# StarsX/FluidX12

Measured on AMD Instinct MI355X. Metric: voxel-updates/sec (advect+40 Jacobi) at 256^3; achieved HBM GB/s vs peak, higher is better.
Workload: dtype f32

## Files before the change

### fluidx12_amd/csrc/fx_jacobi_strip4.hip

```cpp
#include "fx_internal.h"
#include "fx_pk.h"
#include <algorithm>
#include <climits>
#include <cstdlib>

namespace fx {

namespace {

#ifndef FX_STRIP4_OUTER_ROWS
#define FX_STRIP4_OUTER_ROWS 3
#endif
constexpr int NRO = FX_STRIP4_OUTER_ROWS;
constexpr int NRI = 8 - NRO;

template <int NR_, bool A_, bool W_, int NW_ = 4, int XS_ = 0, bool NT_ = false, bool XT_ = false> struct Role4 {
	static constexpr int NR = NR_;
	static constexpr bool XT = XT_;
	static constexpr bool NT = NT_;
	static constexpr int NW = NW_;
	static constexpr int XS = XS_;
	static constexpr int XO1 = 0, XO2 = (A_ || W_) ? 4 : 2, XO3 = (A_ || W_) ? 3 : 4;
	static constexpr bool A = A_, W = W_;
	static constexpr int NI = NR + (A ? 4 : 1) + (W ? 4 : 1);
// ... 35 lines not shown
	fx_f2 lx = XS == 2 ? pk_mov_sel<HI, 0>(E, c01) : pk_mov(c01, c01, 0);
	const fx_f2 mid = pk_mov(c01, c23, 1);
	fx_f2 rx = XS == 1 ? pk_mov_sel<1, HI>(c23, E) : pk_mov(c23, c23, 2);
	const float cx_ = c.x, cw_ = c.w, lx0_ = lx.x, rx1_ = rx.y;
	lx.x = __builtin_bit_cast(float, __builtin_amdgcn_update_dpp(__builtin_bit_cast(int, lx0_), __builtin_bit_cast(int, cw_), 0x138, 0xf, 0xf, false));
	rx.y = __builtin_bit_cast(float, __builtin_amdgcn_update_dpp(__builtin_bit_cast(int, rx1_), __builtin_bit_cast(int, cx_), 0x130, 0xf, 0xf, false));
	const fx_f2 b01 = { bb.x, bb.y }, b23 = { bb.z, bb.w }, U01 = { U.x, U.y }, U23 = { U.z, U.w }, D01 = { D.x, D.y }, D23 = { D.z, D.w };
	const fx_f2 F01 = { F.x, F.y }, F23 = { F.z, F.w }, B01 = { Bk.x, Bk.y }, B23 = { Bk.z, Bk.w };
	fx_f2 s01 = (((((lx - b01) + mid) + U01) + D01) + F01) + B01;
	fx_f2 s23 = (((((mid - b23) + rx) + U23) + D23) + F23) + B23;
	const float inv = __uint_as_float(0x3e2aaaabu);
	s01 *= inv; s23 *= inv;
	return v4f{ s01.x, s01.y, s23.x, s23.y };
}
template <int XS, int C>
__device__ __forceinline__ v4f relax4qe(v4f c, v4f U, v4f D, v4f F, v4f Bk, v4f bb, v4f EA, fx_f2 EB)
{
	static_assert(C >= 0 && C < 6, "six cut cells per step");
	const fx_f2 E = C < 2 ? fx_f2{ EA.x, EA.y } : C < 4 ? fx_f2{ EA.z, EA.w } : EB;
	return relax4qx<XS, C & 1>(c, U, D, F, Bk, bb, E);
}

__device__ __forceinline__ uint32_t opaque32q(uint32_t v) { asm volatile("" : "+v"(v)); return v; }
typedef __attribute__((address_space(1))) v4f g_v4f;
__device__ __forceinline__ void store_row4(char* base, uint32_t off, v4f v)
{
#ifdef FX_S4_SC1
	*(volatile g_v4f*)(g_v4f*)(base + off) = v;
#elif defined(FX_S4_NT)
	__builtin_nontemporal_store(v, reinterpret_cast<v4f*>(base + off));
#else
	*reinterpret_cast<v4f*>(base + off) = v;
#endif
}
__device__ __forceinline__ void store_row4nt(char* base, uint32_t off, v4f v)
{
	__builtin_nontemporal_store(v, reinterpret_cast<v4f*>(base + off));
}

typedef unsigned u4 __attribute__((ext_vector_type(4)));
template <bool NT>
__device__ __forceinline__ void store_row4xt(char* base, uint32_t off, bool keep, v4f v)
{
	const __amdgpu_buffer_rsrc_t rs = __builtin_amdgcn_make_buffer_rsrc(base, 0, 0x7fffffff, 0x00020000);
	const uint32_t o = keep ? off : 0xfffffff0u;
	__builtin_amdgcn_raw_buffer_store_b128(__builtin_bit_cast(u4, v), rs, (int)o, 0, NT ? 2 : 0);
// ... 80 lines not shown
	uint32_t act;
};

__device__ unsigned g_strip4_fault;
constexpr int kWaitSpins4 = 1 << 16;
__device__ __forceinline__ void strip4_raise_fault() { (void)__hip_atomic_fetch_or(&g_strip4_fault, 1u, __ATOMIC_RELAXED, __HIP_MEMORY_SCOPE_AGENT); }

__device__ __forceinline__ v4f lds_wait_read4(uint32_t flag_byte_addr, int need, uint32_t row_byte_addr)
{
	int f;
	v4f d;
	for (int spins = 0;; ++spins) {
		asm volatile("ds_read_b32 %0, %2\n\tds_read_b128 %1, %3\n\ts_waitcnt lgkmcnt(0)" : "=&v"(f), "=&v"(d) : "v"(flag_byte_addr), "v"(row_byte_addr) : "memory");
		if (f >= need) break;
		if (__builtin_expect(spins > kWaitSpins4, 0)) { strip4_raise_fault(); break; }
		__builtin_amdgcn_s_sleep(1);
	}
	return d;
}
__device__ __forceinline__ void lds_post4(uint32_t lds_byte_addr, int v)
{
	asm volatile("ds_write_b32 %0, %1" :: "v"(lds_byte_addr), "v"(v) : "memory");
}

template <class R> struct Strip4 {
	int s_ctr, s_old, s_b2, s_b3, s_b4;
	const char* pp; const char* pbq; char* po; char* po_zb;
	size_t plane_bytes;
	v4f* lds; v4f* xbuf; int* xflag;
	uint32_t xf0, xb0;
	int q, zb, ze, q_load_last, b_load_last, Zg, wave, lane;
	bool wall_top, wall_bot;
	bool keep;
	uint32_t eoff;
	float E0;
	v4f* xe;
	uint32_t xe0;
};
template <int NW> __device__ __forceinline__ constexpr int xeslot(int par, int w) { return (par * NW + w) * 2; }

template <int XS>
__device__ __forceinline__ void xe_publish(uint32_t slot_addr, uint32_t cnt_addr, int q, float v0, float v1, float v2, float v3, float v4, float v5)
{
	if (XS == 1)
		asm volatile("s_bfm_b64 exec, 1, 63\n\tds_write2_b32 %0, %2, %3 offset1:1\n\tds_write2_b32 %0, %4, %5 offset0:2 offset1:3\n\tds_write2_b32 %0, %6, %7 offset0:4 offset1:5\n\t"
			"ds_write_b32 %1, %8\n\ts_mov_b64 exec, -1" :: "v"(slot_addr), "v"(cnt_addr), "v"(v0), "v"(v1), "v"(v2), "v"(v3), "v"(v4), "v"(v5), "v"(q) : "memory");
	else
		asm volatile("s_mov_b64 exec, 1\n\tds_write2_b32 %0, %2, %3 offset1:1\n\tds_write2_b32 %0, %4, %5 offset0:2 offset1:3\n\tds_write2_b32 %0, %6, %7 offset0:4 offset1:5\n\t"
			"ds_write_b32 %1, %8\n\ts_mov_b64 exec, -1" :: "v"(slot_addr), "v"(cnt_addr), "v"(v0), "v"(v1), "v"(v2), "v"(v3), "v"(v4), "v"(v5), "v"(q) : "memory");
}
struct XMail { int f; v4f a; fx_f2 b; };
template <class R>
__device__ __forceinline__ void xe_fetch(const Strip4<R>& st, XMail& x)
// ... 2 lines not shown
	x.f = INT_MAX; return;
#endif
	const int wp = st.wave ^ 4, pr = (st.q - 1) & 1;
	x.f = __hip_atomic_load(reinterpret_cast<const int*>(st.xflag) + 3 * R::NW + wp, __ATOMIC_RELAXED, __HIP_MEMORY_SCOPE_WORKGROUP);
	asm volatile("" ::: "memory");
	__builtin_amdgcn_sched_barrier(0);
	x.a = st.xe[xeslot<R::NW>(pr, wp)];
	x.b = *reinterpret_cast<const fx_f2*>(st.xe + xeslot<R::NW>(pr, wp) + 1);
	asm volatile("" ::: "memory");
	__builtin_amdgcn_sched_barrier(0);
}
template <class R>
__device__ __forceinline__ void xe_check(const Strip4<R>& st, XMail& x)
{
	if (__builtin_expect(x.f < st.q - 1, 0)) {
		const int wp = st.wave ^ 4, pr = (st.q - 1) & 1;
		x.a = lds_wait_read4(st.xf0 + 4u * (uint32_t)(3 * R::NW + wp), st.q - 1, st.xe0 + 16u * (uint32_t)xeslot<R::NW>(pr, wp));
		x.b = *reinterpret_cast<const fx_f2*>(st.xe + xeslot<R::NW>(pr, wp) + 1);
	}
}
__device__ __forceinline__ float lane_cell(float v, int lane) { return __builtin_bit_cast(float, __builtin_amdgcn_readlane(__builtin_bit_cast(int, v), lane)); }

#define FXQ_LDS(st, slot, r) (st).lds[(slot) + (r) * 64]
#define FXQ_RARE_BRANCH asm volatile("; rare path")

template <class R> struct Mail4 { int fu, fd; v4f hu, hd; };

template <class R, int L>
__device__ __forceinline__ void mail_fetch4(const Strip4<R>& st, Mail4<R>& m)
{
#ifdef FX_S4_NOHAND
	return;
#endif
	const int q = st.q, w = st.wave, pr = (q - 1) & 1;
#ifdef FX_S4_BARRIER
	if (!R::A) m.hu = st.xbuf[xrow<R::NW>(pr, FX_WU(w), L - 1, 0) + st.lane];
	if (!R::W) m.hd = st.xbuf[xrow<R::NW>(pr, w, L - 1, 1) + st.lane];
	m.fu = m.fd = INT_MAX;
	return;
#endif
	const int* flags = reinterpret_cast<const int*>(st.xflag);
	if (!R::A) m.fu = __hip_atomic_load(flags + (L - 1) * R::NW + FX_WU(w), __ATOMIC_RELAXED, __HIP_MEMORY_SCOPE_WORKGROUP);
	if (!R::W) m.fd = __hip_atomic_load(flags + (L - 1) * R::NW + FX_WD(w), __ATOMIC_RELAXED, __HIP_MEMORY_SCOPE_WORKGROUP);
	asm volatile("" ::: "memory");
	__builtin_amdgcn_sched_barrier(0);
	if (!R::A) m.hu = st.xbuf[xrow<R::NW>(pr, FX_WU(w), L - 1, 0) + st.lane];
	if (!R::W) m.hd = st.xbuf[xrow<R::NW>(pr, w, L - 1, 1) + st.lane];
	asm volatile("" ::: "memory");
	__builtin_amdgcn_sched_barrier(0);
}

template <class R, int L, int NL>
__device__ __forceinline__ void hand_over4(const Strip4<R>& st, Mail4<R>& m, const v4f (&PN)[NL], v4f& HU, v4f& HD)
{
#ifdef FX_S4_NOHAND
	return;
#endif
	const int q = st.q, w = st.wave;
	const int pr = (q - 1) & 1, pw = q & 1;
	const v4f mine_top = PN[0], mine_bot = PN[NL - 1];
	if (!R::A) {
		if (__builtin_expect(m.fu < q - 1, 0)) m.hu = lds_wait_read4(st.xf0 + 4u * (uint32_t)((L - 1) * R::NW + FX_WU(w)), q - 1, st.xb0 + 16u * (uint32_t)(xrow<R::NW>(pr, FX_WU(w), L - 1, 0) + st.lane));
		HU = m.hu;
	}
	if (!R::W) {
		if (__builtin_expect(m.fd < q - 1, 0)) m.hd = lds_wait_read4(st.xf0 + 4u * (uint32_t)((L - 1) * R::NW + FX_WD(w)), q - 1, st.xb0 + 16u * (uint32_t)(xrow<R::NW>(pr, w, L - 1, 1) + st.lane));
		HD = m.hd;
	}
	asm volatile("" ::: "memory");
	if (!R::A) st.xbuf[xrow<R::NW>(pw, FX_WU(w), L - 1, 1) + st.lane] = mine_top;
	if (!R::W) st.xbuf[xrow<R::NW>(pw, w, L - 1, 0) + st.lane] = mine_bot;
#ifndef FX_S4_BARRIER
#ifdef FX_LAB_DROP_PUBLISH
	if (L == 2 && w == 3) return;
#endif
	if (st.lane == 0) lds_post4(st.xf0 + 4u * (uint32_t)((L - 1) * R::NW + w), q);
#endif
}

template <class R, int L, int NL, int NN, bool MK = false>
__device__ __forceinline__ void relax_level4(const Strip4<R>& st, const v4f (&Pold)[NL], const v4f (&Pctr)[NL], const v4f (&Pnew)[NL],
	const v4f (&Bq)[NN], v4f HU, v4f HD, v4f (&out)[NN], uint32_t mctr, uint32_t& mout, const XMail* xm = nullptr)
{
	constexpr int EOFF = L == 1 ? R::XO1 : L == 2 ? R::XO2 : R::XO3;
	static_assert(!(MK && R::XS), "the masked loop runs on whole-row waves");
	uint32_t m_ = 0u;
#pragma unroll
	for (int kk = 0; kk < NN; ++kk) {
		constexpr int UP = R::UP;
#ifdef FX_M_PLAIN
		const int k = kk;
#else
		const int k = MK ? NN - 1 - kk : kk;
#endif
		const int jc = k + UP;
		const v4f c = Pctr[jc];
		v4f u = jc >= 1 ? Pctr[jc >= 1 ? jc - 1 : 0] : HU;
		v4f d = jc + 1 < NL ? Pctr[jc + 1 < NL ? jc + 1 : 0] : HD;
		if (R::A && k == 3 - L && st.wall_top) u = c;
// ... 10 lines not shown
			switch (k) {
			case 0: out[k] = relax4qe<R::XS ? R::XS : 1, (EOFF + 0) % 6>(c, u, d, Pold[jc], Pnew[jc], Bq[k], xm->a, xm->b); break;
			case 1: out[k] = relax4qe<R::XS ? R::XS : 1, (EOFF + 1) % 6>(c, u, d, Pold[jc], Pnew[jc], Bq[k], xm->a, xm->b); break;
			default: out[k] = relax4qe<R::XS ? R::XS : 1, (EOFF + 2) % 6>(c, u, d, Pold[jc], Pnew[jc], Bq[k], xm->a, xm->b); break;
			}
		} else
			out[k] = relax4q(c, u, d, Pold[jc], Pnew[jc], Bq[k]);
	}
#ifdef FX_M_PLAIN
	if (MK) mout = m_;
#else
	if (MK) mout = ((mctr >> (4 * R::UP)) & ((1u << (4 * NN)) - 1u)) | m_;
#endif
}

template <class R>
__device__ __forceinline__ void frz_out4(const Strip4<R>& st, Frz4& fz, char* dst_, const v4f (&X_)[R::NR], uint32_t m4_, const uint32_t (&roff)[R::NI])
{
	constexpr int NR = R::NR, RB = R::A ? 4 : 1;
	const int z = st.q - 4;
	const ptrdiff_t mo_ = (dst_ - fz.outA) >> 4;
#ifndef FX_M_ONEP
#pragma unroll
	for (int m = 0; m < NR; ++m) store_row4(dst_ + fz.dB, opaque32q(roff[m + RB]), X_[m]);
#endif
#ifdef FX_M_NOBYTES
	if (st.q < -1000)
#endif
#pragma unroll
	for (int m = 0; m < NR; ++m) {
		const uint32_t o_ = opaque32q(roff[m + RB] >> 4);
		fz.mA[mo_ + o_] = (uint8_t)FXQ_NIB(m4_, m);
		fz.mB[mo_ + o_] = (uint8_t)FXQ_NIB(m4_, m);
	}
	if (z >= st.zb) {
#pragma unroll
		for (int m = 0; m < NR; ++m) if (FXQ_NIB(m4_, m) != 15u) { fz.rel |= 16u; fz.act |= 1u << m; }
		if ((z & 7) == 7 || z == st.ze - 1) {
#pragma unroll
			for (int m = 0; m < NR; ++m) {
				const unsigned long long bal_ = __ballot((fz.act >> m) & 1u);
				if ((st.lane & 7) == 0 && ((bal_ >> st.lane) & 0xFFull) != 0ull)
					fz.tile_mark[((z >> 3) * fz.nty + ((fz.y_own + m) >> 3)) * fz.ntx + (st.lane >> 3)] = fz.tag;
			}
			fz.act = 0u;
		}
	}
// ... 2 lines not shown
template <class R, int PH, bool S1, bool S2, bool S3, bool S4, bool MK = false>
__device__ __forceinline__ void step4(Strip4<R>& st, v4f (&P1)[3][R::N1], v4f (&P2)[3][R::N2], v4f (&P3)[3][R::N3], v4f (&NP)[R::NI], v4f (&NB)[R::N1], v4f (&NBn)[R::N1], v4f (&Bk)[R::N2], const uint32_t (&roff)[R::NI],
	Frz4& fz, uint32_t (&MW)[3][3], uint32_t (&NM)[R::N1])
{
	constexpr int NEW = PH % 3, CTR = (PH + 2) % 3, OLD = (PH + 1) % 3;
	constexpr int NI = R::NI, N1 = R::N1, N2 = R::N2, N3 = R::N3, NR = R::NR, UP = R::UP;
	static_assert(!MK || R::NW != 4, "the masked loop runs in the octet");
	constexpr int O1 = R::A ? 3 : 0, O2 = R::A ? 2 : 0, O3 = R::A ? 1 : 0;
	constexpr uint32_t OWN = (1u << (4 * NR)) - 1u;
	const int q = st.q;
	uint32_t M0n = 0u;
	if (MK) {
#pragma unroll
		for (int j = 0; j < N1; ++j) M0n |= (NM[j] & 15u) << (4 * j);
		if (q >= st.zb && q < st.ze && (~(M0n >> (4 * O1)) & OWN) != 0u) fz.rel |= 1u;
		if (q == 0) fz.M0c = M0n;
	}
	const v4f zero = v4f{ 0.0f, 0.0f, 0.0f, 0.0f };
	Mail4<R> M1, M2, M3;
	M1.fu = M1.fd = M2.fu = M2.fd = M3.fu = M3.fd = INT_MIN; M1.hu = M1.hd = M2.hu = M2.hd = M3.hu = M3.hd = zero;
#ifdef FX_S4_BARRIER
	asm volatile("s_waitcnt lgkmcnt(0)\n\ts_barrier" ::: "memory");
#endif
	if (S1) mail_fetch4<R, 1>(st, M1);
	XMail xm; xm.f = INT_MIN; xm.a = zero; xm.b = fx_f2{ 0.0f, 0.0f };
	if (R::XS && S2) xe_fetch<R>(st, xm);
#ifdef FX_S4_LATE_PREFETCH
	constexpr bool EARLY = false;
#else
	constexpr bool EARLY = R::NW == 4;
#endif
	constexpr bool LEAN = R::NW != 4;
	v4f NPc[EARLY ? NI : 1], NBc[EARLY ? N1 : 1];
	auto issue_prefetch = [&]() __attribute__((always_inline)) {
		if (!LEAN) {
#pragma unroll
			for (int j = 0; j < N1; ++j) NB[j] = NBn[j];
		}
#ifdef FX_S4_NOLOAD
		if (q + 1 <= st.b_load_last && q < -1000) {
#else
		if (LEAN ? q <= st.b_load_last : q + 1 <= st.b_load_last) {
#endif
#pragma unroll
			for (int j = 0; j < N1; ++j) (LEAN ? NB[j] : NBn[j]) = *reinterpret_cast<const v4f*>(st.pbq + opaque32q(roff[j + 1]));
		}
#ifdef FX_S4_NOLOAD
		if (q + 1 <= st.q_load_last && q < -1000) {
#else
		if (q + 1 <= st.q_load_last) {
#endif
#pragma unroll
			for (int i = 0; i < NI; ++i) NP[i] = *reinterpret_cast<const v4f*>(st.pp + opaque32q(roff[i]));
			if (MK) {
#pragma unroll
				for (int j = 0; j < N1; ++j) NM[j] = fz.pm[opaque32q(roff[j + 1] >> 4)];
			}
		}
		if (R::XS && q <= st.q_load_last) st.E0 = *reinterpret_cast<const float*>(st.pp - st.plane_bytes + st.eoff);
	};
	if (EARLY) {
#pragma unroll
		for (int i = 0; i < NI; ++i) NPc[i] = NP[i];
#pragma unroll
		for (int j = 0; j < N1; ++j) NBc[j] = NB[j];
		issue_prefetch();
	}
	auto np = [&](int i) __attribute__((always_inline)) -> v4f { return EARLY ? NPc[EARLY ? i : 0] : NP[i]; };
	auto nb = [&](int j) __attribute__((always_inline)) -> v4f { return EARLY ? NBc[EARLY ? j : 0] : NB[j]; };
	if (q == 0) {
#pragma unroll
		for (int i = 0; i < NI; ++i) FXQ_LDS(st, st.s_ctr, i) = np(i);
	}
	fx_f2 E1_[R::XS ? (N1 + 1) / 2 : 1];
	if (R::XS) {
#pragma unroll
		for (int j = 0; j < N1; ++j) { const float e_ = lane_cell(st.E0, j + 1); if (j & 1) E1_[j >> 1].y = e_; else E1_[j >> 1].x = e_; }
	}
	if (S1) {
		v4f T_[N1];
// ... 131 lines not shown
		}
#pragma unroll
		for (int m = 0; m < N3; ++m) P3[NEW][m] = T_[m];
		if (MK) MW[2][NEW] = m3_;
		if (__builtin_expect(q - 3 == 0, 0)) {
			FXQ_RARE_BRANCH;
#pragma unroll
			for (int m = 0; m < N3; ++m) P3[CTR][m] = T_[m];
			if (MK) MW[2][CTR] = m3_;
		}
	}
	v4f HU3 = zero, HD3 = zero;
	if (S3) hand_over4<R, 3, N3>(st, M3, P3[NEW], HU3, HD3);
	if (S4) {
		v4f X_[NR];
		uint32_t m4_ = 0u;
		relax_level4<R, 3, N3, NR, MK>(st, P3[OLD], P3[CTR], P3[NEW], B4_, HU3, HD3, X_, MK ? MW[2][CTR] : 0u, m4_, &xm);
		char* dst_ = q - 4 >= st.zb ? st.po : st.po_zb;
#ifdef FX_S4_NOSTORE
		if (q < -1000)
#endif
#pragma unroll
		for (int m = 0; m < NR; ++m) {
			if (R::XT) store_row4xt<R::NT>(dst_, opaque32q(roff[m + (R::A ? 4 : 1)]), st.keep, X_[m]);
			else if (R::NT) store_row4nt(dst_, opaque32q(roff[m + (R::A ? 4 : 1)]), X_[m]);
			else store_row4(dst_, opaque32q(roff[m + (R::A ? 4 : 1)]), X_[m]);
		}
		if (MK) frz_out4<R>(st, fz, dst_, X_, m4_, roff);
	}
#ifndef FX_S4_NOXE
	if (R::XS) {
		float v_[6] = { 0.0f, 0.0f, 0.0f, 0.0f, 0.0f, 0.0f };
#pragma unroll
		for (int k = 0; k < N2; ++k) v_[R::XO1 + k] = R::XS == 1 ? P1[NEW][k + UP].w : P1[NEW][k + UP].x;
#pragma unroll
		for (int k = 0; k < N3; ++k) v_[R::XO2 + k] = R::XS == 1 ? P2[NEW][k + UP].w : P2[NEW][k + UP].x;
#pragma unroll
		for (int k = 0; k < NR; ++k) v_[R::XO3 + k] = R::XS == 1 ? P3[NEW][k + UP].w : P3[NEW][k + UP].x;
		xe_publish<R::XS ? R::XS : 1>(st.xe0 + 16u * (uint32_t)xeslot<R::NW>(q & 1, st.wave), st.xf0 + 4u * (uint32_t)(3 * R::NW + st.wave), q, v_[0], v_[1], v_[2], v_[3], v_[4], v_[5]);
	}
#endif
	st.po += st.plane_bytes;
	++st.q;
}

template <class R, bool MK>
__device__ __forceinline__ void head_stores4(const Strip4<R>& st, const Frz4& fz, const uint32_t (&roff)[R::NI])
{
#ifndef FX_S4_NOHEADSTORES
	constexpr int RB = R::A ? 4 : 1;
	const v4f zero = v4f{ 0.0f, 0.0f, 0.0f, 0.0f };
#pragma unroll
	for (int m = 0; m < R::NR; ++m) {
		if (R::XT) store_row4xt<false>(st.po_zb, opaque32q(roff[m + RB]), st.keep, zero);
		else store_row4(st.po_zb, opaque32q(roff[m + RB]), zero);
	}
	if (MK) {
		const ptrdiff_t mo_ = (st.po_zb - fz.outA) >> 4;
#pragma unroll
		for (int m = 0; m < R::NR; ++m) store_row4(st.po_zb + fz.dB, opaque32q(roff[m + RB]), zero);
#pragma unroll
		for (int m = 0; m < R::NR; ++m) {
			const uint32_t o_ = opaque32q(roff[m + RB] >> 4);
			fz.mA[mo_ + o_] = (uint8_t)0;
			fz.mB[mo_ + o_] = (uint8_t)0;
		}
	}
#endif
}

template <class R, int NM_>
__device__ __forceinline__ void frz_begin4(const Geom& g, const FrzArgs& fa, const Strip4<R>& st, Frz4& fz, uint32_t (&MW)[3][3], uint32_t (&NM)[NM_],
	const uint32_t (&roff)[R::NI], float* p_out, int y0, int q0, bool fill)
{
	const size_t plane4 = st.plane_bytes >> 4;
	fz.outA = reinterpret_cast<char*>(p_out); fz.dB = reinterpret_cast<char*>(fa.p_outB) - reinterpret_cast<char*>(p_out);
	fz.mA = fa.m_outA; fz.mB = fa.m_outB; fz.tile_mark = fa.tile_mark; fz.tag = fa.tag; fz.ntx = fa.ntx; fz.nty = fa.nty; fz.y_own = y0;
	fz.M0c = 0u; fz.rel = 0u; fz.act = 0u;
#pragma unroll
	for (int l = 0; l < 3; ++l) MW[l][0] = MW[l][1] = MW[l][2] = 0u;
	const uint8_t* mb = fa.m_in + (size_t)g.lz(min(q0, st.q_load_last)) * plane4;
#pragma unroll
	for (int j = 0; j < NM_; ++j) NM[j] = mb[roff[j + 1] >> 4];
// ... 14 lines not shown
__device__ __forceinline__ void run4(const Geom& g, const float* __restrict__ p_in, const float* __restrict__ b, float* __restrict__ p_out,
	int zb, int ze, int y0, int wave, int lane, v4f* lds_slice, v4f* xbuf, int* xflag, const FrzArgs& fa, v4f* xe = nullptr, int x0 = 0, bool keep = true)
{
	Strip4<R> st;
	Frz4 fz;
	uint32_t MW[3][3], NM[R::N1];
#ifndef FX_O_NOPRIO
#ifndef FX_O_PRIO
#define FX_O_PRIO 2
#endif
	if (R::NW != 4) __builtin_amdgcn_s_setprio(FX_O_PRIO);
#endif
	v4f P1[3][R::N1], P2[3][R::N2], P3[3][R::N3], NP[R::NI], NB[R::N1], NBn[R::N1], Bk[R::N2];
	uint32_t roff[R::NI];
	const v4f zero = v4f{ 0.0f, 0.0f, 0.0f, 0.0f };
	const int qs = max(zb - 4, g.zlo), q_last = ze - 1 + 4;
	st.q_load_last = min(q_last, g.zhi);
	st.b_load_last = min(q_last - 1, g.zhi);
	st.zb = zb; st.ze = ze; st.Zg = g.Zg; st.wave = wave; st.lane = lane;
	st.wall_top = y0 == 0; st.wall_bot = y0 + R::NR >= g.Y;
	st.lds = lds_slice + lane; st.xbuf = xbuf; st.xflag = xflag;
	st.xf0 = (uint32_t)(size_t)(__attribute__((address_space(3))) int*)xflag;
	st.xb0 = (uint32_t)(size_t)(__attribute__((address_space(3))) v4f*)xbuf;
	const int yb = y0 - (R::A ? 4 : 1);
	const uint32_t XCOL = R::XT ? (uint32_t)x0 : R::XS == 2 ? 256u : 0u;
	st.keep = keep;
#pragma unroll
	for (int i = 0; i < R::NI; ++i) roff[i] = ((uint32_t)min(max(yb + i, 0), g.Y - 1) * (uint32_t)g.X + XCOL + 4u * (uint32_t)lane) * 4u;
	st.xe = xe; st.xe0 = (uint32_t)(size_t)(__attribute__((address_space(3))) v4f*)xe;
	st.eoff = ((uint32_t)min(max(yb + min(lane, R::NI - 1), 0), g.Y - 1) * (uint32_t)g.X + (R::XS == 2 ? 255u : 256u)) * 4u;
	st.E0 = 0.0f;
	st.s_ctr = 0; st.s_old = R::NI * 64;
	st.s_b2 = 2 * R::NI * 64; st.s_b3 = st.s_b2 + (R::NW == 4 ? R::N2 * 64 : 0); st.s_b4 = st.s_b3 + R::N2 * 64;
#pragma unroll
	for (int k = 0; k < 3; ++k) {
#pragma unroll
		for (int i = 0; i < R::N1; ++i) P1[k][i] = zero;
#pragma unroll
		for (int i = 0; i < R::N2; ++i) P2[k][i] = zero;
#pragma unroll
		for (int i = 0; i < R::N3; ++i) P3[k][i] = zero;
	}
#pragma unroll
	for (int i = 0; i < R::LDS_ROWS; ++i) st.lds[i * 64] = zero;
#pragma unroll
	for (int k = 0; k < R::N2; ++k) Bk[k] = zero;
// ... 9 lines not shown
#pragma unroll
		for (int j = 0; j < R::N1; ++j) NB[j] = *reinterpret_cast<const v4f*>(bbase + roff[j + 1]);
		const char* bnext = reinterpret_cast<const char*>(b + (size_t)g.lz(min(max(q0, g.zlo), g.zhi)) * plane);
#pragma unroll
		for (int j = 0; j < R::N1; ++j) NBn[j] = *reinterpret_cast<const v4f*>(bnext + roff[j + 1]);
		if (R::XS) st.E0 = *reinterpret_cast<const float*>(reinterpret_cast<const char*>(p_in + (size_t)g.lz(min(max(q0 - 1, g.zlo), g.zhi)) * plane) + st.eoff);
		if (fill) {
			const char* pa = reinterpret_cast<const char*>(p_in + (size_t)g.lz(qs) * plane);
			v4f A_[R::NI], B_[R::NI];
#pragma unroll
			for (int i = 0; i < R::NI; ++i) A_[i] = *reinterpret_cast<const v4f*>(pa + roff[i]);
#pragma unroll
			for (int i = 0; i < R::NI; ++i) B_[i] = *reinterpret_cast<const v4f*>(pa + st.plane_bytes + roff[i]);
#pragma unroll
			for (int i = 0; i < R::NI; ++i) FXQ_LDS(st, st.s_old, i) = A_[i];
#pragma unroll
			for (int i = 0; i < R::NI; ++i) FXQ_LDS(st, st.s_ctr, i) = B_[i];
		}
	}
	st.q = q0;
	st.pp = reinterpret_cast<const char*>(p_in) + ((ptrdiff_t)g.lz(q0) + 1) * (ptrdiff_t)st.plane_bytes;
	st.pbq = reinterpret_cast<const char*>(b) + ((ptrdiff_t)g.lz(q0) + (R::NW == 4 ? 1 : 0)) * (ptrdiff_t)st.plane_bytes;
	st.po_zb = reinterpret_cast<char*>(p_out) + (ptrdiff_t)g.lz(zb) * (ptrdiff_t)st.plane_bytes;
	st.po = reinterpret_cast<char*>(p_out) + ((ptrdiff_t)g.lz(q0) - 4) * (ptrdiff_t)st.plane_bytes;
	if (MK) frz_begin4<R, R::N1>(g, fa, st, fz, MW, NM, roff, p_out, y0, q0, fill);
	if (fill) {
		step4<R, 0, true, false, false, false, MK>(st, P1, P2, P3, NP, NB, NBn, Bk, roff, fz, MW, NM);
		step4<R, 1, true, false, false, false, MK>(st, P1, P2, P3, NP, NB, NBn, Bk, roff, fz, MW, NM);
		step4<R, 2, true, true, false, false, MK>(st, P1, P2, P3, NP, NB, NBn, Bk, roff, fz, MW, NM);
		step4<R, 0, true, true, false, false, MK>(st, P1, P2, P3, NP, NB, NBn, Bk, roff, fz, MW, NM);
		step4<R, 1, true, true, true, false, MK>(st, P1, P2, P3, NP, NB, NBn, Bk, roff, fz, MW, NM);
		step4<R, 2, true, true, true, false, MK>(st, P1, P2, P3, NP, NB, NBn, Bk, roff, fz, MW, NM);
	}
	head_stores4<R, MK>(st, fz, roff);
	for (;;) {
		step4<R, 0, true, true, true, true, MK>(st, P1, P2, P3, NP, NB, NBn, Bk, roff, fz, MW, NM);
		if (st.q > q_last) break;
		step4<R, 1, true, true, true, true, MK>(st, P1, P2, P3, NP, NB, NBn, Bk, roff, fz, MW, NM);
		if (st.q > q_last) break;
		step4<R, 2, true, true, true, true, MK>(st, P1, P2, P3, NP, NB, NBn, Bk, roff, fz, MW, NM);
		if (st.q > q_last) break;
	}
	if (MK) frz_end4(fa, fz, lane);
}

template <class R, int PH, bool S1, bool S2, bool S3, bool S4, bool MK = false>
__device__ __forceinline__ void step4r(Strip4<R>& st, v4f (&I)[3][R::NI], v4f (&P1)[3][R::NR], v4f (&P2)[3][R::NR], v4f (&P3)[3][R::NR],
	v4f (&NB)[R::NR], v4f (&Bp)[3][R::NR], const uint32_t (&roff)[R::NI], Frz4& fz, uint32_t (&MW)[3][3], uint32_t (&NM)[R::NR])
{
	static_assert(!R::A && !R::W, "the register-window step serves inner waves");
	constexpr int NEW = PH % 3, CTR = (PH + 2) % 3, OLD = (PH + 1) % 3;
	constexpr int NI = R::NI, NR = R::NR;
	constexpr uint32_t OWN = (1u << (4 * NR)) - 1u;
	const int q = st.q;
	uint32_t M0n = 0u;
	if (MK) {
#pragma unroll
		for (int j = 0; j < NR; ++j) M0n |= (NM[j] & 15u) << (4 * j);
		if (q >= st.zb && q < st.ze && (~M0n & OWN) != 0u) fz.rel |= 1u;
		if (q == 0) fz.M0c = M0n;
	}
	const v4f zero = v4f{ 0.0f, 0.0f, 0.0f, 0.0f };
	Mail4<R> M1, M2, M3;
	M1.fu = M1.fd = M2.fu = M2.fd = M3.fu = M3.fd = INT_MIN; M1.hu = M1.hd = M2.hu = M2.hd = M3.hu = M3.hd = zero;
	if (S1) mail_fetch4<R, 1>(st, M1);
	XMail xm; xm.f = INT_MIN; xm.a = zero; xm.b = fx_f2{ 0.0f, 0.0f };
	if (R::XS && S2) xe_fetch<R>(st, xm);
	if (__builtin_expect(q == 0, 0)) {
		FXQ_RARE_BRANCH;
#pragma unroll
		for (int i = 0; i < NI; ++i) I[CTR][i] = I[NEW][i];
	}
	fx_f2 E1_[R::XS ? (NR + 1) / 2 : 1];
	if (R::XS) {
#pragma unroll
		for (int j = 0; j < NR; ++j) { const float e_ = lane_cell(st.E0, j + 1); if (j & 1) E1_[j >> 1].y = e_; else E1_[j >> 1].x = e_; }
	}
	if (S1) {
		v4f T_[NR];
		uint32_t m1_ = 0u;
		{
#pragma unroll
			for (int jj = 0; jj < NR; ++jj) {
#ifdef FX_M_PLAIN
				const int j = jj;
#else
				const int j = MK ? NR - 1 - jj : jj;
// ... 19 lines not shown
		}
		if (__builtin_expect(q - 1 == st.Zg, 0)) {
			FXQ_RARE_BRANCH;
#pragma unroll
			for (int j = 0; j < NR; ++j) T_[j] = P1[CTR][j];
			if (MK) m1_ = MW[0][CTR];
		}
#pragma unroll
		for (int j = 0; j < NR; ++j) P1[NEW][j] = T_[j];
		if (MK) MW[0][NEW] = m1_;
		if (__builtin_expect(q - 1 == 0, 0)) {
			FXQ_RARE_BRANCH;
#pragma unroll
			for (int j = 0; j < NR; ++j) P1[CTR][j] = T_[j];
			if (MK) MW[0][CTR] = m1_;
		}
	}
	if (MK) fz.M0c = M0n;
	v4f B2_[NR], B3_[NR], B4_[NR];
#pragma unroll
	for (int j = 0; j < NR; ++j) { B2_[j] = Bp[NEW][j]; B3_[j] = Bp[CTR][j]; B4_[j] = Bp[OLD][j]; }
#pragma unroll
	for (int j = 0; j < NR; ++j) Bp[OLD][j] = NB[j];
#ifdef FX_S4_NOLOAD
	if (q + 1 <= st.q_load_last && q < -1000) {
#else
	if (q + 1 <= st.q_load_last) {
#endif
#pragma unroll
		for (int i = 0; i < NI; ++i) I[OLD][i] = *reinterpret_cast<const v4f*>(st.pp + opaque32q(roff[i]));
		if (MK) {
#pragma unroll
			for (int j = 0; j < NR; ++j) NM[j] = fz.pm[opaque32q(roff[j + 1] >> 4)];
		}
	} else {
#pragma unroll
		for (int i = 0; i < NI; ++i) I[OLD][i] = I[NEW][i];
	}
#ifdef FX_S4_NOLOAD
	if (q <= st.b_load_last && q < -1000) {
#else
	if (q <= st.b_load_last) {
#endif
#pragma unroll
		for (int j = 0; j < NR; ++j) NB[j] = *reinterpret_cast<const v4f*>(st.pbq + opaque32q(roff[j + 1]));
	}
	if (R::XS && q <= st.q_load_last) st.E0 = *reinterpret_cast<const float*>(st.pp - st.plane_bytes + st.eoff);
	st.pp += st.plane_bytes; st.pbq += st.plane_bytes;
	if (MK) fz.pm += st.plane_bytes >> 4;
	v4f HU1 = zero, HD1 = zero;
	if (S1) hand_over4<R, 1, NR>(st, M1, P1[NEW], HU1, HD1);
	if (R::XS && S2) xe_check<R>(st, xm);
	if (S2) mail_fetch4<R, 2>(st, M2);
	if (S2) {
		v4f T_[NR];
		uint32_t m2_ = 0u;
		relax_level4<R, 1, NR, NR, MK>(st, P1[OLD], P1[CTR], P1[NEW], B2_, HU1, HD1, T_, MK ? MW[0][CTR] : 0u, m2_, &xm);
		if (MK && q - 2 >= st.zb && q - 2 < st.ze && (~m2_ & OWN) != 0u) fz.rel |= 4u;
		if (__builtin_expect(q - 2 == st.Zg, 0)) {
			FXQ_RARE_BRANCH;
#pragma unroll
			for (int k = 0; k < NR; ++k) T_[k] = P2[CTR][k];
			if (MK) m2_ = MW[1][CTR];
		}
#pragma unroll
		for (int k = 0; k < NR; ++k) P2[NEW][k] = T_[k];
		if (MK) MW[1][NEW] = m2_;
		if (__builtin_expect(q - 2 == 0, 0)) {
// ... 19 lines not shown
		}
#pragma unroll
		for (int m = 0; m < NR; ++m) P3[NEW][m] = T_[m];
		if (MK) MW[2][NEW] = m3_;
		if (__builtin_expect(q - 3 == 0, 0)) {
			FXQ_RARE_BRANCH;
#pragma unroll
			for (int m = 0; m < NR; ++m) P3[CTR][m] = T_[m];
			if (MK) MW[2][CTR] = m3_;
		}
	}
	v4f HU3 = zero, HD3 = zero;
	if (S3) hand_over4<R, 3, NR>(st, M3, P3[NEW], HU3, HD3);
	if (S4) {
		v4f X_[NR];
		uint32_t m4_ = 0u;
		relax_level4<R, 3, NR, NR, MK>(st, P3[OLD], P3[CTR], P3[NEW], B4_, HU3, HD3, X_, MK ? MW[2][CTR] : 0u, m4_, &xm);
		char* dst_ = q - 4 >= st.zb ? st.po : st.po_zb;
#ifdef FX_S4_NOSTORE
		if (q < -1000)
#endif
#pragma unroll
		for (int m = 0; m < NR; ++m) {
			if (R::XT) store_row4xt<R::NT>(dst_, opaque32q(roff[m + 1]), st.keep, X_[m]);
			else if (R::NT) store_row4nt(dst_, opaque32q(roff[m + 1]), X_[m]);
			else store_row4(dst_, opaque32q(roff[m + 1]), X_[m]);
		}
		if (MK) frz_out4<R>(st, fz, dst_, X_, m4_, roff);
	}
#ifndef FX_S4_NOXE
	if (R::XS) {
		float v_[6] = { 0.0f, 0.0f, 0.0f, 0.0f, 0.0f, 0.0f };
#pragma unroll
		for (int k = 0; k < NR; ++k) {
			v_[R::XO1 + k] = R::XS == 1 ? P1[NEW][k].w : P1[NEW][k].x;
			v_[R::XO2 + k] = R::XS == 1 ? P2[NEW][k].w : P2[NEW][k].x;
			v_[R::XO3 + k] = R::XS == 1 ? P3[NEW][k].w : P3[NEW][k].x;
		}
		xe_publish<R::XS ? R::XS : 1>(st.xe0 + 16u * (uint32_t)xeslot<R::NW>(q & 1, st.wave), st.xf0 + 4u * (uint32_t)(3 * R::NW + st.wave), q, v_[0], v_[1], v_[2], v_[3], v_[4], v_[5]);
	}
#endif
	st.po += st.plane_bytes;
	++st.q;
}

template <class R, bool MK = false>
__device__ __forceinline__ void run4r(const Geom& g, const float* __restrict__ p_in, const float* __restrict__ b, float* __restrict__ p_out,
	int zb, int ze, int y0, int wave, int lane, v4f* xbuf, int* xflag, const FrzArgs& fa, v4f* xe = nullptr, int x0 = 0, bool keep = true)
{
	Strip4<R> st;
	Frz4 fz;
	uint32_t MW[3][3], NM[R::NR];
	v4f I[3][R::NI], P1[3][R::NR], P2[3][R::NR], P3[3][R::NR], NB[R::NR], Bp[3][R::NR];
	uint32_t roff[R::NI];
	const v4f zero = v4f{ 0.0f, 0.0f, 0.0f, 0.0f };
	const int qs = max(zb - 4, g.zlo), q_last = ze - 1 + 4;
	st.q_load_last = min(q_last, g.zhi);
	st.b_load_last = min(q_last - 1, g.zhi);
	st.zb = zb; st.ze = ze; st.Zg = g.Zg; st.wave = wave; st.lane = lane;
	st.wall_top = false; st.wall_bot = false;
	st.lds = nullptr; st.xbuf = xbuf; st.xflag = xflag;
	st.xf0 = (uint32_t)(size_t)(__attribute__((address_space(3))) int*)xflag;
	st.xb0 = (uint32_t)(size_t)(__attribute__((address_space(3))) v4f*)xbuf;
	st.s_ctr = st.s_old = st.s_b2 = st.s_b3 = st.s_b4 = 0;
	const int yb = y0 - 1;
	const uint32_t XCOL = R::XT ? (uint32_t)x0 : R::XS == 2 ? 256u : 0u;
	st.keep = keep;
#pragma unroll
	for (int i = 0; i < R::NI; ++i) roff[i] = ((uint32_t)min(max(yb + i, 0), g.Y - 1) * (uint32_t)g.X + XCOL + 4u * (uint32_t)lane) * 4u;
	st.xe = xe; st.xe0 = (uint32_t)(size_t)(__attribute__((address_space(3))) v4f*)xe;
	st.eoff = ((uint32_t)min(max(yb + min(lane, R::NI - 1), 0), g.Y - 1) * (uint32_t)g.X + (R::XS == 2 ? 255u : 256u)) * 4u;
	st.E0 = 0.0f;
#pragma unroll
	for (int k = 0; k < 3; ++k) {
#pragma unroll
		for (int i = 0; i < R::NR; ++i) { P1[k][i] = zero; P2[k][i] = zero; P3[k][i] = zero; Bp[k][i] = zero; }
#pragma unroll
		for (int i = 0; i < R::NI; ++i) I[k][i] = zero;
	}
	const size_t plane = g.plane();
	st.plane_bytes = plane * 4;
	const bool fill = qs == zb - 4;
	const int q0 = fill ? qs + 2 : qs;
	{
		const char* pb = reinterpret_cast<const char*>(p_in + (size_t)g.lz(min(q0, st.q_load_last)) * plane);
#pragma unroll
		for (int i = 0; i < R::NI; ++i) I[0][i] = *reinterpret_cast<const v4f*>(pb + roff[i]);
		const char* bbase = reinterpret_cast<const char*>(b + (size_t)g.lz(min(max(q0 - 1, g.zlo), g.zhi)) * plane);
#pragma unroll
		for (int j = 0; j < R::NR; ++j) NB[j] = *reinterpret_cast<const v4f*>(bbase + roff[j + 1]);
		if (R::XS) st.E0 = *reinterpret_cast<const float*>(reinterpret_cast<const char*>(p_in + (size_t)g.lz(min(max(q0 - 1, g.zlo), g.zhi)) * plane) + st.eoff);
		if (fill) {
			const char* pa = reinterpret_cast<const char*>(p_in + (size_t)g.lz(qs) * plane);
#pragma unroll
			for (int i = 0; i < R::NI; ++i) I[1][i] = *reinterpret_cast<const v4f*>(pa + roff[i]);
#pragma unroll
			for (int i = 0; i < R::NI; ++i) I[2][i] = *reinterpret_cast<const v4f*>(pa + st.plane_bytes + roff[i]);
		}
	}
	st.q = q0;
	st.pp = reinterpret_cast<const char*>(p_in) + ((ptrdiff_t)g.lz(q0) + 1) * (ptrdiff_t)st.plane_bytes;
	st.pbq = reinterpret_cast<const char*>(b) + (ptrdiff_t)g.lz(q0) * (ptrdiff_t)st.plane_bytes;
	st.po_zb = reinterpret_cast<char*>(p_out) + (ptrdiff_t)g.lz(zb) * (ptrdiff_t)st.plane_bytes;
	st.po = reinterpret_cast<char*>(p_out) + ((ptrdiff_t)g.lz(q0) - 4) * (ptrdiff_t)st.plane_bytes;
	if (MK) frz_begin4<R, R::NR>(g, fa, st, fz, MW, NM, roff, p_out, y0, q0, fill);
	if (fill) {
		step4r<R, 0, true, false, false, false, MK>(st, I, P1, P2, P3, NB, Bp, roff, fz, MW, NM);
		step4r<R, 1, true, false, false, false, MK>(st, I, P1, P2, P3, NB, Bp, roff, fz, MW, NM);
		step4r<R, 2, true, true, false, false, MK>(st, I, P1, P2, P3, NB, Bp, roff, fz, MW, NM);
		step4r<R, 0, true, true, false, false, MK>(st, I, P1, P2, P3, NB, Bp, roff, fz, MW, NM);
		step4r<R, 1, true, true, true, false, MK>(st, I, P1, P2, P3, NB, Bp, roff, fz, MW, NM);
		step4r<R, 2, true, true, true, false, MK>(st, I, P1, P2, P3, NB, Bp, roff, fz, MW, NM);
	}
	head_stores4<R, MK>(st, fz, roff);
	for (;;) {
		step4r<R, 0, true, true, true, true, MK>(st, I, P1, P2, P3, NB, Bp, roff, fz, MW, NM);
		if (st.q > q_last) break;
		step4r<R, 1, true, true, true, true, MK>(st, I, P1, P2, P3, NB, Bp, roff, fz, MW, NM);
		if (st.q > q_last) break;
		step4r<R, 2, true, true, true, true, MK>(st, I, P1, P2, P3, NB, Bp, roff, fz, MW, NM);
		if (st.q > q_last) break;
	}
	if (MK) frz_end4(fa, fz, lane);
}

typedef Role4<1, true, false, 8> OctTop;
// ... 422 lines not shown
```

Before: 22.89 billion.

## Precompute LDS mailbox bases and make steady-state plane loads branchless

Precomputes per-wave LDS mailbox flag and row base addresses and toggles them by step parity, so the in-loop address arithmetic shrinks and flag posts use a constant-offset ds_write. For non-4-wave roles without mask, the next-plane loads become unconditional by clamping to a precomputed last-plane pointer, which removes the branches around the global loads. The opaque register pin changes to a by-reference form that keeps row offsets in place. It also merges the two rare-path handoff wait checks into one test. The cost is extra redundant loads at the tail and somewhat more register state.

New measurement: 22.69 billion. Within noise of the previous version (-0.9%).

```diff
diff --git a/fluidx12_amd/csrc/fx_jacobi_strip4.hip b/fluidx12_amd/csrc/fx_jacobi_strip4.hip
--- a/fluidx12_amd/csrc/fx_jacobi_strip4.hip
+++ b/fluidx12_amd/csrc/fx_jacobi_strip4.hip
@@ -81,6 +81,7 @@
 }
 
 __device__ __forceinline__ uint32_t opaque32q(uint32_t v) { asm volatile("" : "+v"(v)); return v; }
+__device__ __forceinline__ uint32_t opaque32k(const uint32_t& v) { uint32_t& r = const_cast<uint32_t&>(v); asm volatile("" : "+v"(r)); return r; }
 typedef __attribute__((address_space(1))) v4f g_v4f;
 __device__ __forceinline__ void store_row4(char* base, uint32_t off, v4f v)
 {
@@ -207,13 +208,20 @@
 {
 	asm volatile("ds_write_b32 %0, %1" :: "v"(lds_byte_addr), "v"(v) : "memory");
 }
+template <int OFF> __device__ __forceinline__ void lds_post4o(uint32_t lds_byte_base, int v)
+{
+	asm volatile("ds_write_b32 %0, %1 offset:%2" :: "v"(lds_byte_base), "v"(v), "n"(OFF) : "memory");
+}
 
 template <class R> struct Strip4 {
 	int s_ctr, s_old, s_b2, s_b3, s_b4;
 	const char* pp; const char* pbq; char* po; char* po_zb;
+	const char* pp_last; const char* pb_last;
 	size_t plane_bytes;
 	v4f* lds; v4f* xbuf; int* xflag;
 	uint32_t xf0, xb0;
+	uint32_t xfw, xrw;
+	uint32_t rin, rout;
 	int q, zb, ze, q_load_last, b_load_last, Zg, wave, lane;
 	bool wall_top, wall_bot;
 	bool keep;
@@ -262,9 +270,53 @@
 __device__ __forceinline__ float lane_cell(float v, int lane) { return __builtin_bit_cast(float, __builtin_amdgcn_readlane(__builtin_bit_cast(int, v), lane)); }
 
 #define FXQ_LDS(st, slot, r) (st).lds[(slot) + (r) * 64]
+#ifdef FX_S4_NOLOAD
+#define FX_RELOAD4(R, MK) false
+#else
+#define FX_RELOAD4(R, MK) ((R::NW != 4) && !(MK))
+#endif
 #define FXQ_RARE_BRANCH asm volatile("; rare path")
 
 template <class R> struct Mail4 { int fu, fd; v4f hu, hd; };
+
+typedef __attribute__((address_space(3))) v4f l_v4f;
+typedef __attribute__((address_space(3))) int l_int;
+template <class R> __device__ __forceinline__ uint32_t mail_rows4(const Strip4<R>& st, int par)
+{
+#ifdef FX_O_ONLYMID
+	return (uint32_t)par;
+#else
+	return st.xrw + (par ? 16u * (uint32_t)xrow<R::NW>(1, 0, 0, 0) : 0u);
+#endif
+}
+template <class R, int L, int SIDE, int DIR> __device__ __forceinline__ uint32_t mail_row4(const Strip4<R>& st, uint32_t rows)
+{
+#ifdef FX_O_ONLYMID
+	return st.xb0 + 16u * (uint32_t)(xrow<R::NW>((int)rows, SIDE ? st.wave : FX_WU(st.wave), L - 1, DIR) + st.lane);
+#else
+	return rows + 16u * (uint32_t)xrow<R::NW>(0, SIDE && !R::A ? 1 : 0, L - 1, DIR);
+#endif
+}
+template <class R, int L, int WHO> __device__ __forceinline__ uint32_t mail_flag4(const Strip4<R>& st)
+{
+#ifdef FX_O_ONLYMID
+	return st.xf0 + 4u * (uint32_t)((L - 1) * R::NW + (WHO == 0 ? FX_WU(st.wave) : WHO == 1 ? st.wave : FX_WD(st.wave)));
+#else
+	return st.xfw + 4u * (uint32_t)((L - 1) * R::NW + WHO - (R::A ? 1 : 0));
+#endif
+}
+template <class R> __device__ __forceinline__ void mail_bases4(Strip4<R>& st)
+{
+	const int w0 = st.wave - (R::A ? 0 : 1);
+	st.xfw = st.xf0 + 4u * (uint32_t)w0;
+	st.xrw = st.xb0 + 16u * (uint32_t)(xrow<R::NW>(0, w0, 0, 0) + st.lane);
+	st.rin = st.rout = st.xrw;
+}
+template <class R> __device__ __forceinline__ void mail_step4(Strip4<R>& st)
+{
+	st.rin = mail_rows4<R>(st, (st.q - 1) & 1);
+	st.rout = mail_rows4<R>(st, st.q & 1);
+}
 
 template <class R, int L>
 __device__ __forceinline__ void mail_fetch4(const Strip4<R>& st, Mail4<R>& m)
@@ -272,20 +324,20 @@
 #ifdef FX_S4_NOHAND
 	return;
 #endif
-	const int q = st.q, w = st.wave, pr = (q - 1) & 1;
+	const l_v4f* const ru = (const l_v4f*)mail_row4<R, L, 0, 0>(st, st.rin);
+	const l_v4f* const rd = (const l_v4f*)mail_row4<R, L, 1, 1>(st, st.rin);
 #ifdef FX_S4_BARRIER
-	if (!R::A) m.hu = st.xbuf[xrow<R::NW>(pr, FX_WU(w), L - 1, 0) + st.lane];
-	if (!R::W) m.hd = st.xbuf[xrow<R::NW>(pr, w, L - 1, 1) + st.lane];
+	if (!R::A) m.hu = *ru;
+	if (!R::W) m.hd = *rd;
 	m.fu = m.fd = INT_MAX;
 	return;
 #endif
-	const int* flags = reinterpret_cast<const int*>(st.xflag);
-	if (!R::A) m.fu = __hip_atomic_load(flags + (L - 1) * R::NW + FX_WU(w), __ATOMIC_RELAXED, __HIP_MEMORY_SCOPE_WORKGROUP);
-	if (!R::W) m.fd = __hip_atomic_load(flags + (L - 1) * R::NW + FX_WD(w), __ATOMIC_RELAXED, __HIP_MEMORY_SCOPE_WORKGROUP);
+	if (!R::A) m.fu = __hip_atomic_load((const l_int*)mail_flag4<R, L, 0>(st), __ATOMIC_RELAXED, __HIP_MEMORY_SCOPE_WORKGROUP);
+	if (!R::W) m.fd = __hip_atomic_load((const l_int*)mail_flag4<R, L, 2>(st), __ATOMIC_RELAXED, __HIP_MEMORY_SCOPE_WORKGROUP);
 	asm volatile("" ::: "memory");
 	__builtin_amdgcn_sched_barrier(0);
-	if (!R::A) m.hu = st.xbuf[xrow<R::NW>(pr, FX_WU(w), L - 1, 0) + st.lane];
-	if (!R::W) m.hd = st.xbuf[xrow<R::NW>(pr, w, L - 1, 1) + st.lane];
+	if (!R::A) m.hu = *ru;
+	if (!R::W) m.hd = *rd;
 	asm volatile("" ::: "memory");
 	__builtin_amdgcn_sched_barrier(0);
 }
@@ -296,25 +348,36 @@
 #ifdef FX_S4_NOHAND
 	return;
 #endif
-	const int q = st.q, w = st.wave;
-	const int pr = (q - 1) & 1, pw = q & 1;
+	const int q = st.q;
 	const v4f mine_top = PN[0], mine_bot = PN[NL - 1];
-	if (!R::A) {
-		if (__builtin_expect(m.fu < q - 1, 0)) m.hu = lds_wait_read4(st.xf0 + 4u * (uint32_t)((L - 1) * R::NW + FX_WU(w)), q - 1, st.xb0 + 16u * (uint32_t)(xrow<R::NW>(pr, FX_WU(w), L - 1, 0) + st.lane));
-		HU = m.hu;
-	}
-	if (!R::W) {
-		if (__builtin_expect(m.fd < q - 1, 0)) m.hd = lds_wait_read4(st.xf0 + 4u * (uint32_t)((L - 1) * R::NW + FX_WD(w)), q - 1, st.xb0 + 16u * (uint32_t)(xrow<R::NW>(pr, w, L - 1, 1) + st.lane));
-		HD = m.hd;
+	if (!R::A && !R::W) {
+		if (__builtin_expect(min(m.fu, m.fd) < q - 1, 0)) {
+			if (m.fu < q - 1) m.hu = lds_wait_read4(mail_flag4<R, L, 0>(st), q - 1, mail_row4<R, L, 0, 0>(st, st.rin));
+			if (m.fd < q - 1) m.hd = lds_wait_read4(mail_flag4<R, L, 2>(st), q - 1, mail_row4<R, L, 1, 1>(st, st.rin));
+		}
+		HU = m.hu; HD = m.hd;
+	} else {
+		if (!R::A) {
+			if (__builtin_expect(m.fu < q - 1, 0)) m.hu = lds_wait_read4(mail_flag4<R, L, 0>(st), q - 1, mail_row4<R, L, 0, 0>(st, st.rin));
+			HU = m.hu;
+		}
+		if (!R::W) {
+			if (__builtin_expect(m.fd < q - 1, 0)) m.hd = lds_wait_read4(mail_flag4<R, L, 2>(st), q - 1, mail_row4<R, L, 1, 1>(st, st.rin));
+			HD = m.hd;
+		}
 	}
 	asm volatile("" ::: "memory");
-	if (!R::A) st.xbuf[xrow<R::NW>(pw, FX_WU(w), L - 1, 1) + st.lane] = mine_top;
-	if (!R::W) st.xbuf[xrow<R::NW>(pw, w, L - 1, 0) + st.lane] = mine_bot;
+	if (!R::A) *(l_v4f*)mail_row4<R, L, 0, 1>(st, st.rout) = mine_top;
+	if (!R::W) *(l_v4f*)mail_row4<R, L, 1, 0>(st, st.rout) = mine_bot;
 #ifndef FX_S4_BARRIER
 #ifdef FX_LAB_DROP_PUBLISH
-	if (L == 2 && w == 3) return;
-#endif
-	if (st.lane == 0) lds_post4(st.xf0 + 4u * (uint32_t)((L - 1) * R::NW + w), q);
+	if (L == 2 && st.wave == 3) return;
+#endif
+#ifdef FX_O_ONLYMID
+	lds_post4(mail_flag4<R, L, 1>(st), q);
+#else
+	lds_post4o<4 * ((L - 1) * R::NW + (R::A ? 0 : 1))>(st.xfw, q);
+#endif
 #endif
 }
 
@@ -371,7 +434,7 @@
 	const ptrdiff_t mo_ = (dst_ - fz.outA) >> 4;
 #ifndef FX_M_ONEP
 #pragma unroll
-	for (int m = 0; m < NR; ++m) store_row4(dst_ + fz.dB, opaque32q(roff[m + RB]), X_[m]);
+	for (int m = 0; m < NR; ++m) store_row4(dst_ + fz.dB, opaque32k(roff[m + RB]), X_[m]);
 #endif
 #ifdef FX_M_NOBYTES
 	if (st.q < -1000)
@@ -420,6 +483,7 @@
 #ifdef FX_S4_BARRIER
 	asm volatile("s_waitcnt lgkmcnt(0)\n\ts_barrier" ::: "memory");
 #endif
+	mail_step4<R>(st);
 	if (S1) mail_fetch4<R, 1>(st, M1);
 	XMail xm; xm.f = INT_MIN; xm.a = zero; xm.b = fx_f2{ 0.0f, 0.0f };
 	if (R::XS && S2) xe_fetch<R>(st, xm);
@@ -435,13 +499,21 @@
 #pragma unroll
 			for (int j = 0; j < N1; ++j) NB[j] = NBn[j];
 		}
+		if (FX_RELOAD4(R, MK)) {
+			const char* const bl_ = q <= st.b_load_last ? st.pbq : st.pb_last;
+#pragma unroll
+			for (int j = 0; j < N1; ++j) NB[j] = *reinterpret_cast<const v4f*>(bl_ + opaque32k(roff[j + 1]));
+			const char* const pl_ = q + 1 <= st.q_load_last ? st.pp : st.pp_last;
+#pragma unroll
+			for (int i = 0; i < NI; ++i) NP[i] = *reinterpret_cast<const v4f*>(pl_ + opaque32k(roff[i]));
+		} else {
 #ifdef FX_S4_NOLOAD
 		if (q + 1 <= st.b_load_last && q < -1000) {
 #else
 		if (LEAN ? q <= st.b_load_last : q + 1 <= st.b_load_last) {
 #endif
 #pragma unroll
-			for (int j = 0; j < N1; ++j) (LEAN ? NB[j] : NBn[j]) = *reinterpret_cast<const v4f*>(st.pbq + opaque32q(roff[j + 1]));
+			for (int j = 0; j < N1; ++j) (LEAN ? NB[j] : NBn[j]) = *reinterpret_cast<const v4f*>(st.pbq + opaque32k(roff[j + 1]));
 		}
 #ifdef FX_S4_NOLOAD
 		if (q + 1 <= st.q_load_last && q < -1000) {
@@ -449,11 +521,12 @@
 		if (q + 1 <= st.q_load_last) {
 #endif
 #pragma unroll
-			for (int i = 0; i < NI; ++i) NP[i] = *reinterpret_cast<const v4f*>(st.pp + opaque32q(roff[i]));
+			for (int i = 0; i < NI; ++i) NP[i] = *reinterpret_cast<const v4f*>(st.pp + opaque32k(roff[i]));
 			if (MK) {
 #pragma unroll
 				for (int j = 0; j < N1; ++j) NM[j] = fz.pm[opaque32q(roff[j + 1] >> 4)];
 			}
+		}
 		}
 		if (R::XS && q <= st.q_load_last) st.E0 = *reinterpret_cast<const float*>(st.pp - st.plane_bytes + st.eoff);
 	};
@@ -631,9 +704,9 @@
 #endif
 #pragma unroll
 		for (int m = 0; m < NR; ++m) {
-			if (R::XT) store_row4xt<R::NT>(dst_, opaque32q(roff[m + (R::A ? 4 : 1)]), st.keep, X_[m]);
-			else if (R::NT) store_row4nt(dst_, opaque32q(roff[m + (R::A ? 4 : 1)]), X_[m]);
-			else store_row4(dst_, opaque32q(roff[m + (R::A ? 4 : 1)]), X_[m]);
+			if (R::XT) store_row4xt<R::NT>(dst_, opaque32k(roff[m + (R::A ? 4 : 1)]), st.keep, X_[m]);
+			else if (R::NT) store_row4nt(dst_, opaque32k(roff[m + (R::A ? 4 : 1)]), X_[m]);
+			else store_row4(dst_, opaque32k(roff[m + (R::A ? 4 : 1)]), X_[m]);
 		}
 		if (MK) frz_out4<R>(st, fz, dst_, X_, m4_, roff);
 	}
@@ -661,13 +734,13 @@
 	const v4f zero = v4f{ 0.0f, 0.0f, 0.0f, 0.0f };
 #pragma unroll
 	for (int m = 0; m < R::NR; ++m) {
-		if (R::XT) store_row4xt<false>(st.po_zb, opaque32q(roff[m + RB]), st.keep, zero);
-		else store_row4(st.po_zb, opaque32q(roff[m + RB]), zero);
+		if (R::XT) store_row4xt<false>(st.po_zb, opaque32k(roff[m + RB]), st.keep, zero);
+		else store_row4(st.po_zb, opaque32k(roff[m + RB]), zero);
 	}
 	if (MK) {
 		const ptrdiff_t mo_ = (st.po_zb - fz.outA) >> 4;
 #pragma unroll
-		for (int m = 0; m < R::NR; ++m) store_row4(st.po_zb + fz.dB, opaque32q(roff[m + RB]), zero);
+		for (int m = 0; m < R::NR; ++m) store_row4(st.po_zb + fz.dB, opaque32k(roff[m + RB]), zero);
 #pragma unroll
 		for (int m = 0; m < R::NR; ++m) {
 			const uint32_t o_ = opaque32q(roff[m + RB] >> 4);
@@ -728,6 +801,7 @@
 	st.lds = lds_slice + lane; st.xbuf = xbuf; st.xflag = xflag;
 	st.xf0 = (uint32_t)(size_t)(__attribute__((address_space(3))) int*)xflag;
 	st.xb0 = (uint32_t)(size_t)(__attribute__((address_space(3))) v4f*)xbuf;
+	mail_bases4<R>(st);
 	const int yb = y0 - (R::A ? 4 : 1);
 	const uint32_t XCOL = R::XT ? (uint32_t)x0 : R::XS == 2 ? 256u : 0u;
 	st.keep = keep;
@@ -783,6 +857,8 @@
 	st.pp = reinterpret_cast<const char*>(p_in) + ((ptrdiff_t)g.lz(q0) + 1) * (ptrdiff_t)st.plane_bytes;
 	st.pbq = reinterpret_cast<const char*>(b) + ((ptrdiff_t)g.lz(q0) + (R::NW == 4 ? 1 : 0)) * (ptrdiff_t)st.plane_bytes;
 	st.po_zb = reinterpret_cast<char*>(p_out) + (ptrdiff_t)g.lz(zb) * (ptrdiff_t)st.plane_bytes;
+	st.pp_last = reinterpret_cast<const char*>(p_in) + (ptrdiff_t)g.lz(st.q_load_last) * (ptrdiff_t)st.plane_bytes;
+	st.pb_last = reinterpret_cast<const char*>(b) + (ptrdiff_t)g.lz(st.b_load_last) * (ptrdiff_t)st.plane_bytes;
 	st.po = reinterpret_cast<char*>(p_out) + ((ptrdiff_t)g.lz(q0) - 4) * (ptrdiff_t)st.plane_bytes;
 	if (MK) frz_begin4<R, R::N1>(g, fa, st, fz, MW, NM, roff, p_out, y0, q0, fill);
 	if (fill) {
@@ -824,6 +900,7 @@
 	const v4f zero = v4f{ 0.0f, 0.0f, 0.0f, 0.0f };
 	Mail4<R> M1, M2, M3;
 	M1.fu = M1.fd = M2.fu = M2.fd = M3.fu = M3.fd = INT_MIN; M1.hu = M1.hd = M2.hu = M2.hd = M3.hu = M3.hd = zero;
+	mail_step4<R>(st);
 	if (S1) mail_fetch4<R, 1>(st, M1);
 	XMail xm; xm.f = INT_MIN; xm.a = zero; xm.b = fx_f2{ 0.0f, 0.0f };
 	if (R::XS && S2) xe_fetch<R>(st, xm);
@@ -889,13 +966,21 @@
 	for (int j = 0; j < NR; ++j) { B2_[j] = Bp[NEW][j]; B3_[j] = Bp[CTR][j]; B4_[j] = Bp[OLD][j]; }
 #pragma unroll
 	for (int j = 0; j < NR; ++j) Bp[OLD][j] = NB[j];
+	if (FX_RELOAD4(R, MK)) {
+		const char* const pl_ = q + 1 <= st.q_load_last ? st.pp : st.pp_last;
+#pragma unroll
+		for (int i = 0; i < NI; ++i) I[OLD][i] = *reinterpret_cast<const v4f*>(pl_ + opaque32k(roff[i]));
+		const char* const bl_ = q <= st.b_load_last ? st.pbq : st.pb_last;
+#pragma unroll
+		for (int j = 0; j < NR; ++j) NB[j] = *reinterpret_cast<const v4f*>(bl_ + opaque32k(roff[j + 1]));
+	} else {
 #ifdef FX_S4_NOLOAD
 	if (q + 1 <= st.q_load_last && q < -1000) {
 #else
 	if (q + 1 <= st.q_load_last) {
 #endif
 #pragma unroll
-		for (int i = 0; i < NI; ++i) I[OLD][i] = *reinterpret_cast<const v4f*>(st.pp + opaque32q(roff[i]));
+		for (int i = 0; i < NI; ++i) I[OLD][i] = *reinterpret_cast<const v4f*>(st.pp + opaque32k(roff[i]));
 		if (MK) {
 #pragma unroll
 			for (int j = 0; j < NR; ++j) NM[j] = fz.pm[opaque32q(roff[j + 1] >> 4)];
@@ -910,7 +995,8 @@
 	if (q <= st.b_load_last) {
 #endif
 #pragma unroll
-		for (int j = 0; j < NR; ++j) NB[j] = *reinterpret_cast<const v4f*>(st.pbq + opaque32q(roff[j + 1]));
+		for (int j = 0; j < NR; ++j) NB[j] = *reinterpret_cast<const v4f*>(st.pbq + opaque32k(roff[j + 1]));
+	}
 	}
 	if (R::XS && q <= st.q_load_last) st.E0 = *reinterpret_cast<const float*>(st.pp - st.plane_bytes + st.eoff);
 	st.pp += st.plane_bytes; st.pbq += st.plane_bytes;
@@ -976,9 +1062,9 @@
 #endif
 #pragma unroll
 		for (int m = 0; m < NR; ++m) {
-			if (R::XT) store_row4xt<R::NT>(dst_, opaque32q(roff[m + 1]), st.keep, X_[m]);
-			else if (R::NT) store_row4nt(dst_, opaque32q(roff[m + 1]), X_[m]);
-			else store_row4(dst_, opaque32q(roff[m + 1]), X_[m]);
+			if (R::XT) store_row4xt<R::NT>(dst_, opaque32k(roff[m + 1]), st.keep, X_[m]);
+			else if (R::NT) store_row4nt(dst_, opaque32k(roff[m + 1]), X_[m]);
+			else store_row4(dst_, opaque32k(roff[m + 1]), X_[m]);
 		}
 		if (MK) frz_out4<R>(st, fz, dst_, X_, m4_, roff);
 	}
@@ -1016,6 +1102,7 @@
 	st.lds = nullptr; st.xbuf = xbuf; st.xflag = xflag;
 	st.xf0 = (uint32_t)(size_t)(__attribute__((address_space(3))) int*)xflag;
 	st.xb0 = (uint32_t)(size_t)(__attribute__((address_space(3))) v4f*)xbuf;
+	mail_bases4<R>(st);
 	st.s_ctr = st.s_old = st.s_b2 = st.s_b3 = st.s_b4 = 0;
 	const int yb = y0 - 1;
 	const uint32_t XCOL = R::XT ? (uint32_t)x0 : R::XS == 2 ? 256u : 0u;
@@ -1056,6 +1143,8 @@
 	st.pp = reinterpret_cast<const char*>(p_in) + ((ptrdiff_t)g.lz(q0) + 1) * (ptrdiff_t)st.plane_bytes;
 	st.pbq = reinterpret_cast<const char*>(b) + (ptrdiff_t)g.lz(q0) * (ptrdiff_t)st.plane_bytes;
 	st.po_zb = reinterpret_cast<char*>(p_out) + (ptrdiff_t)g.lz(zb) * (ptrdiff_t)st.plane_bytes;
+	st.pp_last = reinterpret_cast<const char*>(p_in) + (ptrdiff_t)g.lz(st.q_load_last) * (ptrdiff_t)st.plane_bytes;
+	st.pb_last = reinterpret_cast<const char*>(b) + (ptrdiff_t)g.lz(st.b_load_last) * (ptrdiff_t)st.plane_bytes;
 	st.po = reinterpret_cast<char*>(p_out) + ((ptrdiff_t)g.lz(q0) - 4) * (ptrdiff_t)st.plane_bytes;
 	if (MK) frz_begin4<R, R::NR>(g, fa, st, fz, MW, NM, roff, p_out, y0, q0, fill);
 	if (fill) {
```
